# codgodtao/TMDiff

Measured on AMD Instinct MI355X. Metric: UNet denoise-steps/sec (8-ch 64x64, batch 32), higher is better.
Workload: dtype f32; 1 GPU; BASELINE configs[1]: batch-32 8-ch 64x64 tiles, DDPM p_sample steps of the T=1000 cosine schedule, channel_multiplier [32,64,128,256], full UNet forward (both branches) + fused DDPM update per step; batch_per_gpu=32, parallelism=batch-parallel x1, weights=key-hashed random init, text_embedding=fixed synthetic 768-d

## Files before the change

include/tmdiff_hip.h:

```cpp
#ifndef TMDIFF_HIP_H
#define TMDIFF_HIP_H

#include <stddef.h>
#include <stdint.h>

#ifdef __cplusplus
extern "C" {
#endif

#define TMDIFF_ABI_VERSION 6

#define TMDIFF_OK 0
#define TMDIFF_E_INVALID (-1)
#define TMDIFF_E_UNSUPPORTED (-2)
#define TMDIFF_E_LAUNCH (-3)

typedef void* tmdiff_stream_t;

int tmdiff_version(void);
const char* tmdiff_last_error_string(void);

typedef struct tmdiff_conv3d_desc {
  int32_t B, N, H, W;
  int32_t Cin, Cout;
// ... 79 lines not shown
int tmdiff_conv3d_wino_pack_weights_multi(const tmdiff_wino_pack_entry* entries_dev, const int32_t* chunk_tensor_dev,
                                          const int32_t* chunk_index_dev, int32_t n_chunks, tmdiff_stream_t stream);
int tmdiff_conv3d_wino_fwd(const tmdiff_conv3d_desc* d, void* workspace, tmdiff_stream_t stream);
int tmdiff_conv3d_wino_fwd_stage(const tmdiff_conv3d_desc* d, void* workspace, int32_t stage, tmdiff_stream_t stream);
int tmdiff_conv3d_wino_fwd_xp(const tmdiff_conv3d_desc* d, void* workspace, int32_t stage, float* xp_out, tmdiff_stream_t stream);
int tmdiff_conv3d_wino_fwd_planes(const tmdiff_conv3d_desc* d, void* workspace, int32_t stage, float* xp_out, int32_t planes,
                                  tmdiff_stream_t stream);

int tmdiff_conv3d_wf_supported(const tmdiff_conv3d_desc* d);
int64_t tmdiff_conv3d_wf_blocks(const tmdiff_conv3d_desc* d);
size_t tmdiff_conv3d_wf_splitk_workspace_bytes(const tmdiff_conv3d_desc* d);
size_t tmdiff_conv3d_wf_workspace_bytes(const tmdiff_conv3d_desc* d);
int32_t tmdiff_conv3d_wf_plan(int32_t B, int32_t Cin, int32_t Cout, int32_t N, int32_t H, int32_t W, int32_t groups, int32_t llm,
                              int64_t* tiles);
int tmdiff_conv3d_wf_fwd(const tmdiff_conv3d_desc* d, void* workspace, tmdiff_stream_t stream);
int tmdiff_conv3d_wfll_supported(const tmdiff_conv3d_desc* d);
size_t tmdiff_conv3d_wfll_packed_bytes(int32_t Cout, int32_t Cin);
int tmdiff_conv3d_wfll_pack_weights(const float* w, float* packed, int32_t Cout, int32_t Cin, float ll_scale,
                                    tmdiff_stream_t stream);
size_t tmdiff_conv3d_wfll_splitk_workspace_bytes(const tmdiff_conv3d_desc* d);
int tmdiff_conv3d_wfll_fwd(const tmdiff_conv3d_desc* d, float ll_scale, tmdiff_stream_t stream);

size_t tmdiff_conv3d_packed_bf16_bytes(int32_t Cout, int32_t Cin, int32_t ksize, int32_t groups);
int tmdiff_conv3d_pack_weights_bf16(const float* w, void* packed, int32_t Cout, int32_t Cin, int32_t ksize,
                                    int32_t groups, tmdiff_stream_t stream);
int tmdiff_conv3d_pack_weights_bf16_dgrad(const float* w, void* packed, int32_t Cout, int32_t Cin, int32_t ksize,
                                          int32_t groups, tmdiff_stream_t stream);
size_t tmdiff_conv3d_bf16_workspace_bytes(const tmdiff_conv3d_desc* d);
int tmdiff_conv3d_fwd_bf16(const tmdiff_conv3d_desc* d, void* workspace, tmdiff_stream_t stream);

// ... 294 lines not shown
```

tmdiff_amd/Hyper_unet_general.py:

```python
import math

import torch
import torch.nn as nn

from . import ops, routing

PROMPTS = ("QB", "WV3", "GF2", "WV2", "WV4")

def synthetic_text_embeddings(seed=1234):
    out = {}
    for k, name in enumerate(PROMPTS):
        g = torch.Generator(device="cpu").manual_seed(seed + k)
        out[name] = torch.randn(1, 768, generator=g)
    return out


class Swish(nn.Module):

    def forward(self, x):
        raise RuntimeError("Swish is fused into the HIP kernels; it is never called as a module")



_MASK_FN = None
# ... 307 lines not shown
                        prep["w_wino"][name] = {}
        if self.compute_dtype == "fp32" and ops.config.ll_compose:
            for blk in ("down1", "down2", "down3"):
                m = self.get_submodule(blk + ".down.Conv_0")
                if ops.ll_conv_supported(m.out_channels, m.in_channels, m.kernel_size[0], m.groups):
                    prep["w_ll"][blk + ".down.Conv_0"] = ops.pack_conv_weight_ll(m.weight.detach().float().contiguous(), 0.5)
                    if ops.config.winograd and ops.config.wfll and m.out_channels % 32 == 0:
                        prep["w_wfll"][blk + ".down.Conv_0"] = ops.pack_conv_weight_wfll(m.weight.detach().float().contiguous(), 0.5)
        shift, scale = self._projection_layers()
        prep["shift_bank"] = _Bank(shift, dev)
        prep["scale_bank"] = _Bank(scale, dev)
        self._prep = prep
        self._cond = None
        return prep

    def _conv(self, P, name, segs, use_bias=True, bias_scale=1.0, bias=None, emit=False, **kw):
        m = self.get_submodule(name)
        if bias is None:
            bias = m.bias.detach() if (use_bias and m.bias is not None) else None
        if emit:
            kw["emit"] = emit
        math = "bf16" if name in P["bf16"] else "fp32"
        if m.kernel_size[0] != 3:
            out = ops.conv3d(segs, P["w"][name], m.out_channels, m.kernel_size[0], groups=m.groups, math=math, bias=bias,
                             bias_scale=bias_scale, **kw)
            return (out, None) if emit is None else out
        ww = P["w_wino"].get(name)

        def packed(planes):
            if planes not in ww:
                ww[planes] = ops.pack_conv_weight_wino(m.weight.detach().float().contiguous(), groups=m.groups, planes=planes)
            return ww[planes]

        def packed_wf():
            if "wf" not in ww:
                ww["wf"] = ops.pack_conv_weight_wino(m.weight.detach().float().contiguous(), groups=m.groups, mode=2, planes=6)
            return ww["wf"]

        weights = ops.ConvWeights(lambda: P["w"][name], packed_wf if ww is not None else None, packed if ww is not None else None)
        out = ops.conv3d_auto(segs, weights, m.out_channels, groups=m.groups, math=math, bias=bias, bias_scale=bias_scale, **kw)
        return (out, None) if emit is None else out

    def _spec(self, P, S, shift=None, scale=None, act=True):
        d = {"act": act}
        if shift is not None:
            d["shift"], d["shift_stride"] = P["shift_bank"].slot(S["shift"], shift)
        if scale is not None:
            d["scale"], d["scale_stride"] = P["scale_bank"].slot(S["scale"], scale)
        return d

    @staticmethod
    def _own(spec):
        return dict(in_act=spec["act"], in_shift=spec.get("shift"), shift_stride=spec.get("shift_stride", 0),
                    in_scale=spec.get("scale"), scale_stride=spec.get("scale_stride", 0))
# ... 37 lines not shown
        if side is not None:
            t1p = self._conv(P, name + ".conv20", [side], keep_y=False, emit=pro21)
        elif pre is not None:
            t1p = self._conv(P, name + ".conv20", [pre], keep_y=False, emit=pro21, x_bf16_shape=shape if pre.dtype == torch.int16 else None)
        else:
            t1p = self._conv(P, name + ".conv20", segs, keep_y=False, emit=pro21, **self._own(pro20))
        if plan.emit_ll:
            y2, yll = self._conv(P, name + ".conv21", [t1p], use_bias=False, residual=res, keep_y=False, emit=dict(emit, ll=True), **rckw)
            return None, y2, yll, plan.s2d
        y, y2 = self._conv(P, name + ".conv21", [t1p], use_bias=False, residual=res, emit=emit,
                           x_bf16_shape=shape if name + ".conv21" in P["bf16"] else None, **rckw)
        return (y, y2, None, plan.s2d) if want_ll else (y, y2)

    def _conv0(self, P, name, x, pre):
        if pre is None:
            return self._conv(P, name + ".Conv_0", [x], in_act=True)
        return self._conv(P, name + ".Conv_0", [pre], x_bf16_shape=tuple(x.shape[2:]) if pre.dtype == torch.int16 else None)

    def _down(self, P, S, name, x, flag, want_high, pre=None, emit=None, fuse=False, xq=None, s2d=False):
        shape = x.shape if x is not None else (*xq.shape[:3], 2 * xq.shape[3], 2 * xq.shape[4])
        plan = self._down_plan(P, name, shape, not want_high, pre is not None and pre.dtype == torch.float32, s2d, fuse)
        pro = self._spec(P, S, shift=None if flag else name + ".Dense_0", scale=name + ".dense1")
        if plan.conv0 == "dwt":
            hll, *bands = self._conv(P, name + ".Conv_0", [pre], keep_y=False, emit=dict(pro, dwt=True))
        elif plan.conv0 is None:
            hh = self._conv0(P, name, x, pre)
        rc2 = {}
        if not ops.config.conv2_after_ll:
            xll = ops.haar_dwt2d(self._conv(P, name + ".Conv_2", [x]), want_high=False, ll_scale=0.5)[0]
        else:
            if xq is None:
                xq = ops.haar_dwt2d(x, want_high=False, ll_scale=0.5)[0]
# ... 242 lines not shown
```

tmdiff_amd/_lib.py:

```python
import ctypes as C
import os

_HERE = os.path.dirname(os.path.abspath(__file__))
LIB_PATH = os.environ.get("TMDIFF_HIP_LIB") or os.path.join(_HERE, "libtmdiff_hip.so")

c_float_p = C.POINTER(C.c_float)
vp = C.c_void_p


class Conv3dDesc(C.Structure):
    _fields_ = [
        ("B", C.c_int32), ("N", C.c_int32), ("H", C.c_int32), ("W", C.c_int32),
        ("Cin", C.c_int32), ("Cout", C.c_int32),
        ("groups", C.c_int32), ("ksize", C.c_int32), ("nseg", C.c_int32),
        ("seg_c", C.c_int32 * 3),
        ("seg_x", vp * 3),
        ("w_packed", vp), ("bias", vp), ("bias_scale", C.c_float),
        ("in_shift", vp), ("in_scale", vp), ("in_shift_stride", C.c_int32), ("in_scale_stride", C.c_int32),
        ("in_mask", vp), ("in_act", C.c_int32),
        ("residual", vp), ("out_scale", C.c_float),
        ("y", vp),
        ("y2", vp), ("y2_shift", vp), ("y2_scale", vp), ("y2_shift_stride", C.c_int32), ("y2_scale_stride", C.c_int32),
        ("y2_act", C.c_int32), ("y2_bf16", C.c_int32), ("x_bf16", C.c_int32),
        ("splitk_ws", vp), ("splitk_ws_bytes", C.c_int64),
# ... 15 lines not shown
    "tmdiff_conv3d_fwd_staged_workspace_bytes": (C.c_size_t, [C.POINTER(Conv3dDesc)]),
    "tmdiff_conv3d_fwd_staged": (C.c_int, [C.POINTER(Conv3dDesc), vp, vp]),
    "tmdiff_conv3d_wino_supported": (C.c_int, [C.POINTER(Conv3dDesc)]),
    "tmdiff_conv3d_wino_blocks": (C.c_int64, [C.POINTER(Conv3dDesc)]),
    "tmdiff_conv3d_wino_workspace_bytes": (C.c_size_t, [C.POINTER(Conv3dDesc)]),
    "tmdiff_conv3d_wino_planes": (C.c_int32, [C.c_int32]),
    "tmdiff_conv3d_wino_packed_bytes": (C.c_size_t, [C.c_int32, C.c_int32, C.c_int32, C.c_int32]),
    "tmdiff_conv3d_wino_pack_weights": (C.c_int, [vp, vp, C.c_int32, C.c_int32, C.c_int32, C.c_int32, C.c_int32, vp]),
    "tmdiff_conv3d_wino_pack_weights_multi_chunk": (C.c_int32, []),
    "tmdiff_conv3d_wino_pack_weights_multi": (C.c_int, [vp, vp, vp, C.c_int32, vp]),
    "tmdiff_conv3d_wf_supported": (C.c_int, [C.POINTER(Conv3dDesc)]),
    "tmdiff_conv3d_wf_blocks": (C.c_int64, [C.POINTER(Conv3dDesc)]),
    "tmdiff_conv3d_wf_workspace_bytes": (C.c_size_t, [C.POINTER(Conv3dDesc)]),
    "tmdiff_conv3d_wf_splitk_workspace_bytes": (C.c_size_t, [C.POINTER(Conv3dDesc)]),
    "tmdiff_conv3d_wf_fwd": (C.c_int, [C.POINTER(Conv3dDesc), vp, vp]),
    "tmdiff_conv3d_wino_fwd": (C.c_int, [C.POINTER(Conv3dDesc), vp, vp]),
    "tmdiff_conv3d_wino_fwd_planes": (C.c_int, [C.POINTER(Conv3dDesc), vp, C.c_int32, vp, C.c_int32, vp]),
    "tmdiff_conv3d_wino_fwd_xp": (C.c_int, [C.POINTER(Conv3dDesc), vp, C.c_int32, vp, vp]),
    "tmdiff_conv3d_wino_fwd_stage": (C.c_int, [C.POINTER(Conv3dDesc), vp, C.c_int32, vp]),
    "tmdiff_conv3d_prologue_fwd": (C.c_int, [C.POINTER(Conv3dDesc), vp, vp]),
    "tmdiff_conv3d_ll_supported": (C.c_int, [C.POINTER(Conv3dDesc)]),
    "tmdiff_conv3d_ll_splitk_workspace_bytes": (C.c_size_t, [C.POINTER(Conv3dDesc)]),
    "tmdiff_conv3d_ll_packed_bytes": (C.c_size_t, [C.c_int32, C.c_int32]),
    "tmdiff_conv3d_ll_pack_weights": (C.c_int, [vp, vp, C.c_int32, C.c_int32, C.c_float, vp]),
    "tmdiff_conv3d_ll_fwd": (C.c_int, [C.POINTER(Conv3dDesc), C.c_float, vp]),
    "tmdiff_conv3d_packed_bf16_bytes": (C.c_size_t, [C.c_int32, C.c_int32, C.c_int32, C.c_int32]),
    "tmdiff_conv3d_pack_weights_bf16": (C.c_int, [vp, vp, C.c_int32, C.c_int32, C.c_int32, C.c_int32, vp]),
    "tmdiff_conv3d_bf16_workspace_bytes": (C.c_size_t, [C.POINTER(Conv3dDesc)]),
    "tmdiff_conv3d_fwd_bf16": (C.c_int, [C.POINTER(Conv3dDesc), vp, vp]),
    "tmdiff_conv3d_wgrad_workspace_bytes": (C.c_size_t, [C.POINTER(Conv3dDesc)]),
# ... 185 lines not shown
```

tmdiff_amd/csrc/bufaddr.h:

```cpp
#pragma once
#include <hip/hip_runtime.h>

namespace tmdiff {
namespace buf {

constexpr unsigned kOutside = 0xFFFFFFF0u;

#if defined(__HIP_DEVICE_COMPILE__)
using rsrc = __amdgpu_buffer_rsrc_t;
__device__ __forceinline__ rsrc make(const void* base, unsigned bytes) {
  return __builtin_amdgcn_make_buffer_rsrc(const_cast<void*>(base), 0, bytes, 0x00020000);
}
using u32x4 = __attribute__((ext_vector_type(4))) unsigned;
using u32x2 = __attribute__((ext_vector_type(2))) unsigned;
__device__ __forceinline__ float load(rsrc r, unsigned voff, unsigned soff) {
  return __uint_as_float(__builtin_amdgcn_raw_buffer_load_b32(r, voff, soff, 0));
}
__device__ __forceinline__ float4 load4(rsrc r, unsigned voff) {
  const u32x4 v = __builtin_amdgcn_raw_buffer_load_b128(r, voff, 0, 0);
  return make_float4(__uint_as_float(v.x), __uint_as_float(v.y), __uint_as_float(v.z), __uint_as_float(v.w));
}
__device__ __forceinline__ void store4(rsrc r, unsigned voff, float4 t) {
  const u32x4 v = {__float_as_uint(t.x), __float_as_uint(t.y), __float_as_uint(t.z), __float_as_uint(t.w)};
  __builtin_amdgcn_raw_buffer_store_b128(v, r, voff, 0, 0);
}
__device__ __forceinline__ void store4(rsrc r, unsigned voff, uint4 t) {
  const u32x4 v = {t.x, t.y, t.z, t.w};
  __builtin_amdgcn_raw_buffer_store_b128(v, r, voff, 0, 0);
}
__device__ __forceinline__ void store2(rsrc r, unsigned voff, float2 t) {
  const u32x2 v = {__float_as_uint(t.x), __float_as_uint(t.y)};
  __builtin_amdgcn_raw_buffer_store_b64(v, r, voff, 0, 0);
}
__device__ __forceinline__ void dma_b128(rsrc r, unsigned voff, unsigned soff, float* dst) {
  __builtin_amdgcn_raw_ptr_buffer_load_lds(r, dst, 16, voff, soff, 0, 0);
}
#else
struct rsrc {};
__device__ __forceinline__ rsrc make(const void*, unsigned) { return {}; }
__device__ __forceinline__ float load(rsrc, unsigned, unsigned) { return 0.f; }
__device__ __forceinline__ float4 load4(rsrc, unsigned) { return make_float4(0.f, 0.f, 0.f, 0.f); }
__device__ __forceinline__ void store4(rsrc, unsigned, float4) {}
__device__ __forceinline__ void store4(rsrc, unsigned, uint4) {}
__device__ __forceinline__ void store2(rsrc, unsigned, float2) {}
__device__ __forceinline__ void dma_b128(rsrc, unsigned, unsigned, float*) {}
#endif
__device__ __forceinline__ unsigned at(unsigned base, unsigned add) { return base >= kOutside ? kOutside : base + add; }

__device__ __forceinline__ void dma_b32(const float* src, float* dst) {
#if defined(__HIP_DEVICE_COMPILE__)
  __builtin_amdgcn_global_load_lds(src, dst, 4, 0, 0);
#endif
}
__device__ __forceinline__ void dma_b128(const float* src, float* dst) {
#if defined(__HIP_DEVICE_COMPILE__)
  __builtin_amdgcn_global_load_lds(src, dst, 16, 0, 0);
// ... 6 lines not shown
```

tmdiff_amd/ops.py:

```python
import collections
import ctypes as C
import math
import os

import numpy as np
import torch

from . import _lib, routing
from ._lib import Conv3dDesc, check, lib



class KernelConfig:

    _FLAG = lambda default: (lambda v: (v != "0") if default else (v == "1"))
    _FIELDS = {
        "winograd": ("TMDIFF_WINOGRAD", _FLAG(True), True), "wf": ("TMDIFF_WF", _FLAG(True), True),
        "wf_pair": ("TMDIFF_WF_PAIR", _FLAG(True), True), "wf_splitk": ("TMDIFF_WF_SPLITK", _FLAG(True), True),
        "wf_min_fill": ("TMDIFF_WF_MIN_FILL", float, 0.7), "wino_min_blocks": ("TMDIFF_WINO_MIN_BLOCKS", int, 256),
        "ll_compose": ("TMDIFF_LL_COMPOSE", _FLAG(True), True), "wfll": ("TMDIFF_WFLL", _FLAG(True), True),
        "train_ll_wino": ("TMDIFF_TRAIN_LL_WINO", _FLAG(True), True),
        "conv2_after_ll": ("TMDIFF_CONV2_AFTER_LL", _FLAG(True), True),
        "epilogue_fuse": ("TMDIFF_EPILOGUE_FUSE", _FLAG(True), True), "producer_fuse": ("TMDIFF_PRODUCER_FUSE", _FLAG(True), True),
        "fp32_staged": ("TMDIFF_FP32_STAGED", str, "auto"), "bf16_pack": ("TMDIFF_BF16_PACK", str, "auto"),
        "wgrad_wino": ("TMDIFF_WGRAD_WINO", _FLAG(True), True), "wgrad_wino_bias": ("TMDIFF_WGRAD_WINO_BIAS", _FLAG(True), True),
        "wgrad_bias": ("TMDIFF_WGRAD_BIAS", _FLAG(False), False), "wino_multipack": ("TMDIFF_WINO_MULTIPACK", _FLAG(True), True),
        "fuse_res_conv": ("TMDIFF_FUSE_RES_CONV", _FLAG(True), True), "emit_ll": ("TMDIFF_EMIT_LL", _FLAG(True), True),
        "emit_dwt": ("TMDIFF_EMIT_DWT", _FLAG(True), True), "side_xp": ("TMDIFF_SIDE_XP", _FLAG(True), True),
        "train_fused_resblock": ("TMDIFF_TRAIN_FUSED_RESBLOCK", _FLAG(True), True),
        "train_graph": ("TMDIFF_TRAIN_GRAPH", _FLAG(False), False),
        "train_two_streams": ("TMDIFF_TRAIN_STREAMS", _FLAG(True), True),
        "sample_graph": ("TMDIFF_SAMPLE_GRAPH", _FLAG(False), False),
        "grad_bf16": ("TMDIFF_GRAD_BF16", _FLAG(False), False),
    }

    def __init__(self, env=None):
        env = os.environ if env is None else env
        for name, (var, parse, default) in self._FIELDS.items():
            object.__setattr__(self, name, parse(env[var]) if var in env else default)

    def __setattr__(self, name, value):
        if name not in self._FIELDS:
            raise AttributeError(f"ops.config has no switch {name!r}")
        object.__setattr__(self, name, value)

    def key(self):
        return tuple(getattr(self, n) for n in self._FIELDS)

# ... 519 lines not shown
        raise ValueError(f"pack_conv_weight_wino: weight shape {tuple(w.shape)} (groups {groups}, mode {mode}, planes {planes}) not supported")
    out = torch.empty(nb // 4, device=w.device, dtype=torch.float32)
    check(lib.tmdiff_conv3d_wino_pack_weights(_chk(w.detach(), "w"), out.data_ptr(), cout, cin, groups, mode, planes, stream_ptr()),
          "conv3d_wino_pack_weights")
    return out


wino_conv_supported = routing.wino_weight_ok
ll_conv_supported = routing.ll_weight_ok
wf_route = routing.wf_route
wfll_route = routing.wfll_route


class ConvWeights:

    def __init__(self, direct, wf=None, wino=None):
        self.direct, self.wf, self.wino = direct, wf, wino


def conv3d_auto(segs, weights, cout, groups=1, math="fp32", emit=None, keep_y=True, xp_out=None, x_bf16_shape=None, family=None,
                **kw):
    if math == "bf16" or x_bf16_shape is not None:
        return conv3d(segs, weights.direct(), cout, 3, groups=groups, math=math, emit=emit, keep_y=keep_y,
                      x_bf16_shape=x_bf16_shape, **kw)
    b, _, n, h, w = segs[0].shape
    cin = sum(s_.shape[1] for s_ in segs)
    masked, dropout, plain = kw.get("in_mask") is not None, kw.get("drop") is not None, _plain(segs, kw)
    fam = family or routing.conv3_family(b, cin, cout, n, h, w, groups, plain=plain, masked=masked, dropout=dropout,
                                         keep_xp=xp_out is not None)
    if fam in ("wf", "wf_pair") and weights.wf is not None:
        return conv3d_wf(segs, weights.wf(), cout, emit=emit, keep_y=keep_y, groups=groups, xp_out=xp_out, **kw)
    if fam in ("wino4", "wino2") and weights.wino is not None:
        from . import fallback
        planes = 6 if fam == "wino4" else 4
        return fallback.conv3d_wino(segs, weights.wino(planes), cout, planes, emit=emit, keep_y=keep_y, groups=groups,
                                    xp_out=xp_out, **kw)
    if (emit is not None and (emit.get("s2d") or emit.get("ll") or emit.get("dwt"))) or kw.get("res_conv") is not None:
        raise ValueError("conv3d_auto: only conv3d_wf writes a space-to-depth second output / folds a residual convolution "
                         "(ask routing.wf_route first)")
    if fam not in ("staged", "fused"):
        fam = routing.direct_family(cin, cout, groups, plain, masked, dropout, xp_out is not None, extents=(b, n, h, w))
    return conv3d(segs, weights.direct(), cout, 3, groups=groups, staged=fam == "staged", emit=emit, keep_y=keep_y,
                  xp_out=xp_out, **kw)

# ... 18 lines not shown
    y_hi = [torch.empty(*q, device=dev, dtype=torch.float32) for _ in range(3)] if want_dwt else None
    y, y2 = _outputs("conv3d_wf", dev, (b, cout, n, h, w), keep_y, emit,
                     None if want_dwt else ((b, 4 * cout, n, h // 2, w // 2) if s2d else (b, cout, n, h, w)))
    d = make_conv_desc(segs, w_packed, cout, 3, y, y2=y2, groups=groups, y2_s2d=s2d, y_ll=y_ll, y_hi=y_hi, **kw,
                       **_emit_kw(emit))
    if not lib.tmdiff_conv3d_wf_supported(C.byref(d)):
        raise ValueError("conv3d_wf: shape not supported")
    _lend_splitk(d, dev, lib.tmdiff_conv3d_wf_splitk_workspace_bytes(C.byref(d)) if (config.wf_splitk and not want_ll) else 0)
    nws = lib.tmdiff_conv3d_wf_workspace_bytes(C.byref(d))
    ws = _xp_target("conv3d_wf", xp_out, nws, dev)
    if xp_out is not None and not nws:
        xp_out.copy_(segs[0] if len(segs) == 1 else torch.cat(segs, 1))
    flops = 2.0 * b * cout * ((d.Cin // groups) * 13.5 + d.rc_cin) * n * h * w
    _launch(lib.tmdiff_conv3d_wf_fwd, d, (ws,), "conv3d_wf_fwd", "conv3d_wf_fwd", flops, 3, f" +rc{d.rc_cin}" if d.rc_cin else "")
    return (y_ll, *y_hi) if want_dwt else (y2, y_ll) if want_ll else _result(y, y2)


def pack_conv_weight_ll(w, ll_scale=0.5):
    cout, cin = w.shape[0], w.shape[1]
    nb = lib.tmdiff_conv3d_ll_packed_bytes(cout, cin)
    if tuple(w.shape[2:]) != (3, 3, 3) or nb == 0:
        raise ValueError(f"pack_conv_weight_ll: weight shape {tuple(w.shape)} not supported")
    out = torch.empty(nb // 4, device=w.device, dtype=torch.float32)
    check(lib.tmdiff_conv3d_ll_pack_weights(_chk(w.detach(), "w"), out.data_ptr(), cout, cin, float(ll_scale), stream_ptr()),
          "conv3d_ll_pack_weights")
    return out


def conv3d_ll(x, w_packed, cout, ll_scale=0.5, emit=None, keep_y=True, **kw):
    b, _, n, h, w = x.shape
# ... 1454 lines not shown
```

tmdiff_amd/routing.py:

```python
import collections
import ctypes as C

from . import _lib
from ._lib import lib

PRODUCT_FAMILIES = ("wf", "wf_pair", "wfll", "ll", "staged", "fused", "bf16")
FALLBACK_FAMILIES = ("wino4", "wino2")


def _config():
    from . import ops
    return ops.config


def _grad_bf16():
    return bool(getattr(_config(), "grad_bf16", False))


def wino_weight_ok(cout, cin, ksize=3, groups=1):
    return (ksize == 3 and groups in (1, 3) and cin % groups == 0 and cout % groups == 0 and (cin // groups) % 2 == 0 and
            (cout // groups) % 32 == 0)


def staged_weight_ok(cout, cin, groups=1):
# ... 44 lines not shown
def supported(query, b, cin, cout, n, h, w, groups=1, **fields):
    key = (query, b, cin, cout, n, h, w, groups, tuple(sorted(fields.items())))
    r = _QUERIES.get(key)
    if r is None:
        if len(_QUERIES) > 4096:
            _QUERIES.clear()
        seg_c = cin if isinstance(cin, tuple) else (cin,)
        d = _lib.Conv3dDesc()
        d.B, d.N, d.H, d.W, d.Cin, d.Cout, d.groups, d.ksize, d.nseg = b, n, h, w, sum(seg_c), cout, groups, 3, len(seg_c)
        for i, c in enumerate(seg_c):
            d.seg_c[i] = c
        for k, v in fields.items():
            setattr(d, k, v)
        r = _QUERIES[key] = bool(getattr(lib, query)(C.byref(d)))
    return r


def wfll_route(b, cin, cout, n, h, w):
    if not (_config().wfll and n in (4, 8) and h % 2 == 0 and w % 8 == 0 and cout % 32 == 0):
        return False
    return wf_route(b, 4 * cin, cout, n, h // 2, w // 2, llm=True)[0]


def wino_plan(b, cout, n, h, w, groups=1, cin=None):
    planes = lib.tmdiff_conv3d_wino_planes(int(n))
    if not planes or w % 4:
        return 0, 0
    if cin is not None and not supported("tmdiff_conv3d_wino_supported", b, cin, cout, n, h, w, groups):
        return 0, 0
    cg = cout // groups
# ... 411 lines not shown
```

Baseline: 45.33 batch32-steps/s.

## Add 2D Winograd F(4,3)xF(2,3) conv path for deep low-resolution layers

Adds a new three-pass convolution for fp32 3x3x3 layers with Cin>=128 and Cout>=256 at small spatial sizes (W<=16, H<=32). It applies Winograd transforms along depth (F(4,3)) and width (F(2,3)), runs 24 batched MFMA GEMMs over channels with double-buffered LDS staging, and does the inverse transform plus bias, residual and activation in an output pass. Routing sends eligible 'wf' family convs there by default. The aim is to cut multiply work on the deep UNet layers, at the cost of extra workspace round-trips through global memory, two more kernel launches per conv, and a one-time weight pack.

New measurement: 46.02 batch32-steps/s (median of 6 runs). +1.5%, better.

```diff
diff --git a/include/tmdiff_hip.h b/include/tmdiff_hip.h
--- a/include/tmdiff_hip.h
+++ b/include/tmdiff_hip.h
@@ -117,6 +117,12 @@
 int32_t tmdiff_conv3d_wf_plan(int32_t B, int32_t Cin, int32_t Cout, int32_t N, int32_t H, int32_t W, int32_t groups, int32_t llm,
                               int64_t* tiles);
 int tmdiff_conv3d_wf_fwd(const tmdiff_conv3d_desc* d, void* workspace, tmdiff_stream_t stream);
+
+int tmdiff_conv3d_w2_supported(const tmdiff_conv3d_desc* d);
+size_t tmdiff_conv3d_w2_workspace_bytes(const tmdiff_conv3d_desc* d);
+size_t tmdiff_conv3d_w2_packed_bytes(int32_t Cout, int32_t Cin);
+int tmdiff_conv3d_w2_pack_weights(const float* w, float* packed, int32_t Cout, int32_t Cin, tmdiff_stream_t stream);
+int tmdiff_conv3d_w2_fwd(const tmdiff_conv3d_desc* d, void* workspace, int32_t stages, tmdiff_stream_t stream);
 int tmdiff_conv3d_wfll_supported(const tmdiff_conv3d_desc* d);
 size_t tmdiff_conv3d_wfll_packed_bytes(int32_t Cout, int32_t Cin);
 int tmdiff_conv3d_wfll_pack_weights(const float* w, float* packed, int32_t Cout, int32_t Cin, float ll_scale,
diff --git a/tmdiff_amd/Hyper_unet_general.py b/tmdiff_amd/Hyper_unet_general.py
--- a/tmdiff_amd/Hyper_unet_general.py
+++ b/tmdiff_amd/Hyper_unet_general.py
@@ -345,7 +345,7 @@
         self._cond = None
         return prep
 
-    def _conv(self, P, name, segs, use_bias=True, bias_scale=1.0, bias=None, emit=False, **kw):
+    def _conv(self, P, name, segs, use_bias=True, bias_scale=1.0, bias=None, emit=False, w2=True, **kw):
         m = self.get_submodule(name)
         if bias is None:
             bias = m.bias.detach() if (use_bias and m.bias is not None) else None
@@ -368,7 +368,13 @@
                 ww["wf"] = ops.pack_conv_weight_wino(m.weight.detach().float().contiguous(), groups=m.groups, mode=2, planes=6)
             return ww["wf"]
 
-        weights = ops.ConvWeights(lambda: P["w"][name], packed_wf if ww is not None else None, packed if ww is not None else None)
+        def packed_w2():
+            if "w2" not in ww:
+                ww["w2"] = ops.pack_conv_weight_w2(m.weight.detach().float().contiguous())
+            return ww["w2"]
+
+        weights = ops.ConvWeights(lambda: P["w"][name], packed_wf if ww is not None else None, packed if ww is not None else None,
+                                  packed_w2 if (w2 and ww is not None and m.groups == 1) else None)
         out = ops.conv3d_auto(segs, weights, m.out_channels, groups=m.groups, math=math, bias=bias, bias_scale=bias_scale, **kw)
         return (out, None) if emit is None else out
 
@@ -436,8 +442,8 @@
 
     def _conv0(self, P, name, x, pre):
         if pre is None:
-            return self._conv(P, name + ".Conv_0", [x], in_act=True)
-        return self._conv(P, name + ".Conv_0", [pre], x_bf16_shape=tuple(x.shape[2:]) if pre.dtype == torch.int16 else None)
+            return self._conv(P, name + ".Conv_0", [x], in_act=True, w2=False)
+        return self._conv(P, name + ".Conv_0", [pre], x_bf16_shape=tuple(x.shape[2:]) if pre.dtype == torch.int16 else None, w2=False)
 
     def _down(self, P, S, name, x, flag, want_high, pre=None, emit=None, fuse=False, xq=None, s2d=False):
         shape = x.shape if x is not None else (*xq.shape[:3], 2 * xq.shape[3], 2 * xq.shape[4])
diff --git a/tmdiff_amd/_lib.py b/tmdiff_amd/_lib.py
--- a/tmdiff_amd/_lib.py
+++ b/tmdiff_amd/_lib.py
@@ -53,6 +53,11 @@
     "tmdiff_conv3d_wf_workspace_bytes": (C.c_size_t, [C.POINTER(Conv3dDesc)]),
     "tmdiff_conv3d_wf_splitk_workspace_bytes": (C.c_size_t, [C.POINTER(Conv3dDesc)]),
     "tmdiff_conv3d_wf_fwd": (C.c_int, [C.POINTER(Conv3dDesc), vp, vp]),
+    "tmdiff_conv3d_w2_supported": (C.c_int, [C.POINTER(Conv3dDesc)]),
+    "tmdiff_conv3d_w2_workspace_bytes": (C.c_size_t, [C.POINTER(Conv3dDesc)]),
+    "tmdiff_conv3d_w2_packed_bytes": (C.c_size_t, [C.c_int32, C.c_int32]),
+    "tmdiff_conv3d_w2_pack_weights": (C.c_int, [vp, vp, C.c_int32, C.c_int32, vp]),
+    "tmdiff_conv3d_w2_fwd": (C.c_int, [C.POINTER(Conv3dDesc), vp, C.c_int32, vp]),
     "tmdiff_conv3d_wino_fwd": (C.c_int, [C.POINTER(Conv3dDesc), vp, vp]),
     "tmdiff_conv3d_wino_fwd_planes": (C.c_int, [C.POINTER(Conv3dDesc), vp, C.c_int32, vp, C.c_int32, vp]),
     "tmdiff_conv3d_wino_fwd_xp": (C.c_int, [C.POINTER(Conv3dDesc), vp, C.c_int32, vp, vp]),
diff --git a/tmdiff_amd/csrc/bufaddr.h b/tmdiff_amd/csrc/bufaddr.h
--- a/tmdiff_amd/csrc/bufaddr.h
+++ b/tmdiff_amd/csrc/bufaddr.h
@@ -20,6 +20,13 @@
   const u32x4 v = __builtin_amdgcn_raw_buffer_load_b128(r, voff, 0, 0);
   return make_float4(__uint_as_float(v.x), __uint_as_float(v.y), __uint_as_float(v.z), __uint_as_float(v.w));
 }
+__device__ __forceinline__ float2 load2(rsrc r, unsigned voff) {
+  const u32x2 v = __builtin_amdgcn_raw_buffer_load_b64(r, voff, 0, 0);
+  return make_float2(__uint_as_float(v.x), __uint_as_float(v.y));
+}
+__device__ __forceinline__ void store(rsrc r, unsigned voff, float t) {
+  __builtin_amdgcn_raw_buffer_store_b32(__float_as_uint(t), r, voff, 0, 0);
+}
 __device__ __forceinline__ void store4(rsrc r, unsigned voff, float4 t) {
   const u32x4 v = {__float_as_uint(t.x), __float_as_uint(t.y), __float_as_uint(t.z), __float_as_uint(t.w)};
   __builtin_amdgcn_raw_buffer_store_b128(v, r, voff, 0, 0);
@@ -40,6 +47,8 @@
 __device__ __forceinline__ rsrc make(const void*, unsigned) { return {}; }
 __device__ __forceinline__ float load(rsrc, unsigned, unsigned) { return 0.f; }
 __device__ __forceinline__ float4 load4(rsrc, unsigned) { return make_float4(0.f, 0.f, 0.f, 0.f); }
+__device__ __forceinline__ float2 load2(rsrc, unsigned) { return make_float2(0.f, 0.f); }
+__device__ __forceinline__ void store(rsrc, unsigned, float) {}
 __device__ __forceinline__ void store4(rsrc, unsigned, float4) {}
 __device__ __forceinline__ void store4(rsrc, unsigned, uint4) {}
 __device__ __forceinline__ void store2(rsrc, unsigned, float2) {}
diff --git a/tmdiff_amd/csrc/conv3d_w2.hip b/tmdiff_amd/csrc/conv3d_w2.hip
--- /dev/null
+++ b/tmdiff_amd/csrc/conv3d_w2.hip
@@ -0,0 +1,438 @@
+#include "bufaddr.h"
+#include "common.h"
+
+namespace {
+
+using namespace tmdiff;
+
+constexpr int W2_XP = 384;
+constexpr int W2_NP = 256;
+constexpr int W2_KC = 16;
+constexpr int W2_CO = 64;
+
+struct W2Plan {
+  int T, Q, TW, Hp, IP, OP;
+  int G, ptiles;
+  size_t xh_floats, mh_floats;
+};
+
+bool w2_shape_ok(const tmdiff_conv3d_desc* d) {
+  if (!d || d->ksize != 3 || d->groups != 1 || d->x_bf16 || d->y2_bf16 || d->nseg != 1) return false;
+  if (d->B <= 0 || (d->N != 4 && d->N != 8) || d->W < 2 || d->W > 16 || d->W % 2 || d->H < 4 || d->H > 32) return false;
+  if (d->Cin < 128 || d->Cin % 32 || d->Cout < 256 || d->Cout % W2_CO || d->seg_c[0] != d->Cin) return false;
+  if (d->in_mask || d->drop_p > 0.f || d->rc_x || d->rc_cin || d->y_ll || d->y_hi[0] || d->y2_s2d || d->xp_out) return false;
+  return true;
+}
+
+W2Plan w2_plan(const tmdiff_conv3d_desc* d) {
+  W2Plan p;
+  p.T = d->N / 4; p.Q = d->B * p.T; p.TW = d->W / 2; p.Hp = d->H + 2;
+  p.IP = p.Hp * p.TW; p.OP = d->H * p.TW;
+  p.G = W2_NP / p.OP < W2_XP / p.IP ? W2_NP / p.OP : W2_XP / p.IP;
+  if (p.G > p.Q) p.G = p.Q;
+  p.ptiles = (p.Q + p.G - 1) / p.G;
+  p.xh_floats = (size_t)24 * d->Cin * p.Q * p.IP;
+  p.mh_floats = (size_t)24 * d->Cout * p.Q * p.OP;
+  return p;
+}
+
+bool w2_fits(const tmdiff_conv3d_desc* d, const W2Plan& p) {
+  const size_t xk = p.xh_floats / 24 * 4, mk = p.mh_floats / 24 * 4, uk = (size_t)3 * d->Cin * d->Cout * 4;
+  return xk < (1ull << 31) && mk < (1ull << 31) && uk < (1ull << 31) && p.Q <= 65535 &&
+         (long)p.ptiles * (d->Cout / W2_CO) * 24 < 0x7fffffffL;
+}
+
+__global__ void __launch_bounds__(256) w2_pack_kernel(const float* __restrict__ w, float* __restrict__ u, int Cout, int Cin) {
+#pragma clang fp contract(off)
+  const long idx = (long)blockIdx.x * 256 + threadIdx.x;
+  if (idx >= (long)3 * Cin * Cout) return;
+  const int e = idx & 3;
+  long r = idx >> 2;
+  const int co = r % Cout; r /= Cout;
+  const int cq = r % (Cin / 4);
+  const int dh = r / (Cin / 4);
+  const int ci = cq * 4 + e;
+  const float* src = w + ((long)co * Cin + ci) * 27 + dh * 3;
+  float t[6][3];
+#pragma unroll
+  for (int dw = 0; dw < 3; ++dw) {
+    const float g0 = src[dw], g1 = src[9 + dw], g2 = src[18 + dw];
+    const float s02 = g0 + g2;
+    const float ev = g0 + 4.f * g2, od = 2.f * g1;
+    t[0][dw] = 0.25f * g0;
+    t[1][dw] = (s02 + g1) * (-1.f / 6.f);
+    t[2][dw] = (g1 - s02) * (1.f / 6.f);
+    t[3][dw] = (ev + od) * (1.f / 24.f);
+    t[4][dw] = (ev - od) * (1.f / 24.f);
+    t[5][dw] = g2;
+  }
+  const long plane = (long)3 * Cin * Cout;
+  float* dst = u + (((long)dh * (Cin / 4) + cq) * Cout + co) * 4 + e;
+#pragma unroll
+  for (int kb = 0; kb < 6; ++kb) {
+    const float s02 = t[kb][0] + t[kb][2];
+    dst[(kb * 4 + 0) * plane] = t[kb][0];
+    dst[(kb * 4 + 1) * plane] = 0.5f * (s02 + t[kb][1]);
+    dst[(kb * 4 + 2) * plane] = 0.5f * (s02 - t[kb][1]);
+    dst[(kb * 4 + 3) * plane] = t[kb][2];
+  }
+}
+
+struct W2InArgs {
+  const float* x;
+  float* xh;
+  const float* in_shift;
+  const float* in_scale;
+  int shift_stride, scale_stride, in_act;
+  int Cin, N, H, W, T, TW, IP;
+  long QIP;
+};
+
+__global__ void __launch_bounds__(256) w2_input_kernel(const W2InArgs a) {
+  __shared__ float tile[24 * 8 * 33];
+  const int tid = threadIdx.x;
+  const int cc = blockIdx.x, hp = blockIdx.y, q = blockIdx.z;
+  const int b = q / a.T, t = q % a.T;
+  const int h = hp - 1;
+  {
+    const int c = tid >> 3, tw = tid & 7;
+    const int ch = cc * 32 + c;
+    const long hw = (long)a.H * a.W;
+    const bool ok = h >= 0 && h < a.H && tw < a.TW;
+    const float sh = a.in_shift ? a.in_shift[(long)b * a.shift_stride + ch] : 0.f;
+    const float sc = a.in_scale ? a.in_scale[(long)b * a.scale_stride + ch] : 1.f;
+    const float* src = a.x + ((long)b * a.Cin + ch) * a.N * hw + (long)h * a.W + 2 * tw;
+    float d[6][4];
+#pragma unroll
+    for (int j = 0; j < 6; ++j) {
+      const int n = 4 * t - 1 + j;
+      float2 v = make_float2(0.f, 0.f);
+      if (ok && n >= 0 && n < a.N) {
+        v = *reinterpret_cast<const float2*>(src + (long)n * hw);
+        v.x += sh, v.y += sh;
+        if (a.in_act) v.x = silu_f(v.x), v.y = silu_f(v.y);
+        v.x *= sc, v.y *= sc;
+      }
+      const float left = __shfl_up(v.y, 1, 8), right = __shfl_down(v.x, 1, 8);
+      d[j][0] = tw == 0 ? 0.f : left;
+      d[j][1] = v.x, d[j][2] = v.y;
+      d[j][3] = tw == 7 ? 0.f : right;
+    }
+    float o[6][4];
+#pragma unroll
+    for (int e = 0; e < 4; ++e) {
+      const float d0 = d[0][e], d1 = d[1][e], d2 = d[2][e], d3 = d[3][e], d4 = d[4][e], d5 = d[5][e];
+      const float a42 = d4 - 4.f * d2, b31 = d3 - 4.f * d1, c42 = d4 - d2, e31 = d3 - d1;
+      o[0][e] = (4.f * d0 + d4) - 5.f * d2;
+      o[1][e] = a42 + b31;
+      o[2][e] = a42 - b31;
+      o[3][e] = c42 + 2.f * e31;
+      o[4][e] = c42 - 2.f * e31;
+      o[5][e] = (4.f * d1 + d5) - 5.f * d3;
+    }
+#pragma unroll
+    for (int kb = 0; kb < 6; ++kb) {
+      float* dst = tile + (kb * 4 * 8 + tw) * 33 + c;
+      dst[0 * 8 * 33] = o[kb][0] - o[kb][2];
+      dst[1 * 8 * 33] = o[kb][1] + o[kb][2];
+      dst[2 * 8 * 33] = o[kb][2] - o[kb][1];
+      dst[3 * 8 * 33] = o[kb][1] - o[kb][3];
+    }
+  }
+  __syncthreads();
+  const int n_out = 24 * 8 * a.TW;
+  const long pos = (long)q * a.IP + (long)hp * a.TW;
+  for (int i = tid; i < n_out; i += 256) {
+    const int tw = i % a.TW, r = i / a.TW;
+    const int cq = r & 7, k = r >> 3;
+    const float* s = tile + (k * 8 + tw) * 33 + cq * 4;
+    float* dst = a.xh + (((long)k * (a.Cin / 4) + cc * 8 + cq) * a.QIP + pos + tw) * 4;
+    *reinterpret_cast<float4*>(dst) = make_float4(s[0], s[1], s[2], s[3]);
+  }
+}
+
+struct W2GemmArgs {
+  const float* xh;
+  const float* u;
+  float* mh;
+  int Cin, Cout, Q, TW, IP, OP, G, ptiles, cotiles;
+  unsigned total_blocks;
+};
+
+__global__ void __launch_bounds__(256, 2) w2_gemm_kernel(const W2GemmArgs a) {
+  constexpr int XS = W2_XP * W2_KC;
+  constexpr int US = 3 * W2_KC * W2_CO;
+  constexpr int STAGE = XS + US;
+  __shared__ __attribute__((aligned(16))) float lds[2 * STAGE];
+  float* const st0 = lds;
+  float* const st1 = lds + STAGE;
+
+  const int tid = threadIdx.x;
+  const int lane = tid & 63, wv = __builtin_amdgcn_readfirstlane(tid >> 6);
+  const int l31 = lane & 31, khalf = lane >> 5;
+
+  unsigned id = xcd_remap(blockIdx.x, a.total_blocks);
+  const int co_t = take(id, a.cotiles);
+  const int p_t = take(id, a.ptiles);
+  const int k = __builtin_amdgcn_readfirstlane(id);
+  const int q0 = p_t * a.G;
+  const int nvalid = min(a.G, a.Q - q0) * a.OP;
+  const long QIP = (long)a.Q * a.IP, QOP = (long)a.Q * a.OP;
+  const long xplane = (long)a.Cin * QIP, uplane = (long)3 * a.Cin * a.Cout, mplane = QOP * a.Cout;
+  const buf::rsrc rx = buf::make(a.xh + (long)k * xplane, (unsigned)(xplane * 4));
+  const buf::rsrc ru = buf::make(a.u + (long)k * uplane, (unsigned)(uplane * 4));
+  const buf::rsrc rm = buf::make(a.mh + (long)k * mplane, (unsigned)(mplane * 4));
+
+  unsigned xv[6], uv[3];
+#pragma unroll
+  for (int c = 0; c < 6; ++c) xv[c] = (unsigned)((q0 * a.IP + c * 64 + lane) * 16);
+  const unsigned quad_bytes = (unsigned)(QIP * 16);
+#pragma unroll
+  for (int i = 0; i < 3; ++i) {
+    const int ui = wv * 3 + i, dh = ui >> 2, qd = ui & 3;
+    uv[i] = (unsigned)((((long)dh * (a.Cin / 4) + qd) * a.Cout + co_t * W2_CO + lane) * 16);
+  }
+  const unsigned ustage_bytes = (unsigned)(4 * a.Cout * 16);
+  auto issue = [&](int s, float* st) __attribute__((always_inline)) {
+    const unsigned xso = (unsigned)(4 * s + wv) * quad_bytes, uso = (unsigned)s * ustage_bytes;
+#pragma unroll
+    for (int c = 0; c < 6; ++c) buf::dma_b128(rx, xv[c], xso, st + (wv * W2_XP + c * 64) * 4);
+#pragma unroll
+    for (int i = 0; i < 3; ++i) buf::dma_b128(ru, uv[i], uso, st + XS + (wv * 3 + i) * 256);
+  };
+
+  int aoff[2][3];
+#pragma unroll
+  for (int pb = 0; pb < 2; ++pb) {
+    int c = (2 * wv + pb) * 32 + l31;
+    if (c >= nvalid) c = 0;
+    const int padded = (c / a.OP) * a.IP + c % a.OP;
+#pragma unroll
+    for (int dh = 0; dh < 3; ++dh) aoff[pb][dh] = (khalf * W2_XP + padded + dh * a.TW) * 4;
+  }
+  const int boff = XS + (khalf * W2_CO + l31) * 4;
+
+  f32x16 acc[2][2];
+#pragma unroll
+  for (int pb = 0; pb < 2; ++pb)
+#pragma unroll
+    for (int cb = 0; cb < 2; ++cb)
+#pragma unroll
+      for (int r = 0; r < 16; ++r) acc[pb][cb][r] = 0.f;
+
+  auto compute = [&](const float* st) __attribute__((always_inline)) {
+    static_for<0, 6>([&](auto ic) __attribute__((always_inline)) {
+      constexpr int dh = decltype(ic)::value / 2, m = decltype(ic)::value % 2;
+      float4 av[2], bv[2];
+#pragma unroll
+      for (int pb = 0; pb < 2; ++pb) av[pb] = *reinterpret_cast<const float4*>(st + aoff[pb][dh] + m * 2 * W2_XP * 4);
+#pragma unroll
+      for (int cb = 0; cb < 2; ++cb)
+        bv[cb] = *reinterpret_cast<const float4*>(st + boff + ((dh * 4 + 2 * m) * W2_CO + cb * 32) * 4);
+#pragma unroll
+      for (int e = 0; e < 4; ++e) {
+        const float a0 = e == 0 ? av[0].x : e == 1 ? av[0].y : e == 2 ? av[0].z : av[0].w;
+        const float a1 = e == 0 ? av[1].x : e == 1 ? av[1].y : e == 2 ? av[1].z : av[1].w;
+        const float b0 = e == 0 ? bv[0].x : e == 1 ? bv[0].y : e == 2 ? bv[0].z : bv[0].w;
+        const float b1 = e == 0 ? bv[1].x : e == 1 ? bv[1].y : e == 2 ? bv[1].z : bv[1].w;
+        acc[0][0] = __builtin_amdgcn_mfma_f32_32x32x2f32(a0, b0, acc[0][0], 0, 0, 0);
+        acc[0][1] = __builtin_amdgcn_mfma_f32_32x32x2f32(a0, b1, acc[0][1], 0, 0, 0);
+        acc[1][0] = __builtin_amdgcn_mfma_f32_32x32x2f32(a1, b0, acc[1][0], 0, 0, 0);
+        acc[1][1] = __builtin_amdgcn_mfma_f32_32x32x2f32(a1, b1, acc[1][1], 0, 0, 0);
+      }
+    });
+  };
+
+  const int ns = a.Cin / W2_KC;
+  issue(0, st0);
+  for (int s = 0; s < ns; s += 2) {
+    __builtin_amdgcn_s_waitcnt(0x0F70);
+    __syncthreads();
+    issue(s + 1, st1);
+    compute(st0);
+    __builtin_amdgcn_s_waitcnt(0x0F70);
+    __syncthreads();
+    if (s + 2 < ns) issue(s + 2, st0);
+    compute(st1);
+  }
+
+#pragma unroll
+  for (int pb = 0; pb < 2; ++pb)
+#pragma unroll
+    for (int r = 0; r < 16; ++r) {
+      const int c = (2 * wv + pb) * 32 + (r & 3) + 8 * (r >> 2) + 4 * khalf;
+      const unsigned o = c < nvalid ? (unsigned)((((long)q0 * a.OP + c) * a.Cout + co_t * W2_CO + l31) * 4) : buf::kOutside;
+      buf::store(rm, o, acc[pb][0][r]);
+      buf::store(rm, buf::at(o, 128u), acc[pb][1][r]);
+    }
+}
+
+struct W2OutArgs {
+  const float* mh;
+  const float* bias;
+  float bias_scale;
+  const float* residual;
+  float out_scale;
+  float* y;
+  float* y2;
+  const float* y2_shift;
+  const float* y2_scale;
+  int y2_shift_stride, y2_scale_stride, y2_act;
+  int Cout, N, H, W, T, TW, OP;
+  long QOP;
+};
+
+template <bool Y, bool RES, bool Y2>
+__global__ void __launch_bounds__(256) w2_output_kernel(const W2OutArgs a) {
+#pragma clang fp contract(off)
+  __shared__ float tile[4 * 32 * 17];
+  const int tid = threadIdx.x;
+  const int cc = blockIdx.x, h = blockIdx.y, q = blockIdx.z;
+  const int b = q / a.T, t = q % a.T;
+  {
+    const int co_l = tid & 31, tw = tid >> 5;
+    if (tw < a.TW) {
+      const float* src = a.mh + ((long)q * a.OP + h * a.TW + tw) * a.Cout + cc * 32 + co_l;
+      const long kstride = a.QOP * a.Cout;
+      float r[6][2];
+#pragma unroll
+      for (int kb = 0; kb < 6; ++kb) {
+        const float m0 = src[(kb * 4 + 0) * kstride], m1 = src[(kb * 4 + 1) * kstride], m2 = src[(kb * 4 + 2) * kstride],
+                    m3 = src[(kb * 4 + 3) * kstride];
+        r[kb][0] = (m0 + m1) + m2;
+        r[kb][1] = (m1 - m2) - m3;
+      }
+#pragma unroll
+      for (int j = 0; j < 2; ++j) {
+        const float p12 = r[1][j] + r[2][j], d12 = r[1][j] - r[2][j], p34 = r[3][j] + r[4][j], d34 = r[3][j] - r[4][j];
+        float* dst = tile + co_l * 17 + 2 * tw + j;
+        dst[0 * 32 * 17] = (r[0][j] + p12) + p34;
+        dst[1 * 32 * 17] = d12 + 2.f * d34;
+        dst[2 * 32 * 17] = p12 + 4.f * p34;
+        dst[3 * 32 * 17] = (d12 + 8.f * d34) + r[5][j];
+      }
+    }
+  }
+  __syncthreads();
+  const long plane = (long)a.N * a.H * a.W;
+  const long cb = ((long)b * a.Cout + cc * 32) * plane;
+  const unsigned span = (unsigned)(32 * plane * 4);
+  const buf::rsrc ry = buf::make(Y ? a.y + cb : nullptr, Y ? span : 0u);
+  const buf::rsrc rr = buf::make(RES ? a.residual + cb : nullptr, RES ? span : 0u);
+  const buf::rsrc r2 = buf::make(Y2 ? a.y2 + cb : nullptr, Y2 ? span : 0u);
+#pragma unroll
+  for (int it = 0; it < 4; ++it) {
+    const int i = tid + 256 * it;
+    const int wp = i & 7, band = (i >> 3) & 3, co_l = i >> 5;
+    const int co = cc * 32 + co_l;
+    const unsigned o = wp < a.TW ? (unsigned)(((co_l * (long)a.N + 4 * t + band) * a.H + h) * a.W + 2 * wp) * 4u : buf::kOutside;
+    const float* s = tile + (band * 32 + co_l) * 17 + 2 * wp;
+    float v[2] = {s[0], s[1]};
+    const float bias_t = a.bias ? a.bias[co] * a.bias_scale : 0.f;
+    float2 res = make_float2(0.f, 0.f);
+    if constexpr (RES) res = buf::load2(rr, o);
+    v[0] = (v[0] + bias_t + res.x) * a.out_scale;
+    v[1] = (v[1] + bias_t + res.y) * a.out_scale;
+    if constexpr (Y) buf::store2(ry, o, make_float2(v[0], v[1]));
+    if constexpr (Y2) {
+      const float sh2 = a.y2_shift ? a.y2_shift[(long)b * a.y2_shift_stride + co] : 0.f;
+      const float sc2 = a.y2_scale ? a.y2_scale[(long)b * a.y2_scale_stride + co] : 1.f;
+      float u[2];
+#pragma unroll
+      for (int e = 0; e < 2; ++e) {
+        const float x = v[e] + sh2;
+        const float xa = silu_f(x);
+        u[e] = (a.y2_act ? xa : x) * sc2;
+      }
+      buf::store2(r2, o, make_float2(u[0], u[1]));
+    }
+  }
+}
+
+}
+
+extern "C" int tmdiff_conv3d_w2_supported(const tmdiff_conv3d_desc* d) {
+  return w2_shape_ok(d) && w2_fits(d, w2_plan(d)) ? 1 : 0;
+}
+
+extern "C" size_t tmdiff_conv3d_w2_workspace_bytes(const tmdiff_conv3d_desc* d) {
+  if (!w2_shape_ok(d)) return 0;
+  const W2Plan p = w2_plan(d);
+  return (p.xh_floats + p.mh_floats) * sizeof(float);
+}
+
+extern "C" size_t tmdiff_conv3d_w2_packed_bytes(int32_t Cout, int32_t Cin) {
+  if (Cout <= 0 || Cin <= 0 || Cin % 4) return 0;
+  return (size_t)72 * Cout * Cin * sizeof(float);
+}
+
+extern "C" int tmdiff_conv3d_w2_pack_weights(const float* w, float* packed, int32_t Cout, int32_t Cin, tmdiff_stream_t stream) {
+  using namespace tmdiff;
+  TMDIFF_REQUIRE(w && packed, "conv3d_w2_pack_weights: NULL pointer");
+  TMDIFF_REQUIRE(Cout > 0 && Cin > 0 && Cin % 4 == 0 && (size_t)72 * Cout * Cin < (1ull << 31),
+                 "conv3d_w2_pack_weights: Cout=%d Cin=%d (Cin %% 4 == 0)", Cout, Cin);
+  const long n = (long)3 * Cin * Cout;
+  w2_pack_kernel<<<(unsigned)((n + 255) / 256), 256, 0, as_stream(stream)>>>(w, packed, Cout, Cin);
+  return check_launch("conv3d_w2_pack_weights");
+}
+
+extern "C" int tmdiff_conv3d_w2_fwd(const tmdiff_conv3d_desc* d, void* workspace, int32_t stages, tmdiff_stream_t stream) {
+  using namespace tmdiff;
+  TMDIFF_REQUIRE(d && workspace, "conv3d_w2_fwd: NULL pointer");
+  if (!w2_shape_ok(d))
+    return fail(TMDIFF_E_UNSUPPORTED, "conv3d_w2_fwd: fp32 3x3x3, groups 1, one input tensor, 4 or 8 bands, even W <= 16, 4 <= H <= 32, "
+                                      "Cin >= 128 (%% 32), Cout >= 256 (%% 64), plain y / y2 / residual epilogue");
+  const W2Plan p = w2_plan(d);
+  if (!w2_fits(d, p)) return fail(TMDIFF_E_UNSUPPORTED, "conv3d_w2_fwd: tensor too large for 32-bit offsets");
+  TMDIFF_REQUIRE(d->seg_x[0] && d->w_packed && (d->y || d->y2), "conv3d_w2_fwd: input, weights and an output");
+  TMDIFF_REQUIRE(aligned16(d->seg_x[0]) && aligned16(workspace) && aligned16(d->w_packed) && aligned16(d->y) && aligned16(d->y2) &&
+                     aligned16(d->residual),
+                 "conv3d_w2_fwd: 16-byte aligned tensors / workspace");
+  hipStream_t st = as_stream(stream);
+  float* xh = static_cast<float*>(workspace);
+  float* mh = xh + p.xh_floats;
+  if (stages == 0) stages = 7;
+
+  if (stages & 1) {
+    W2InArgs a;
+    a.x = d->seg_x[0]; a.xh = xh;
+    a.in_shift = d->in_shift; a.in_scale = d->in_scale;
+    a.shift_stride = bank_stride(d->in_shift_stride, d->Cin);
+    a.scale_stride = bank_stride(d->in_scale_stride, d->Cin);
+    a.in_act = d->in_act;
+    a.Cin = d->Cin; a.N = d->N; a.H = d->H; a.W = d->W; a.T = p.T; a.TW = p.TW; a.IP = p.IP;
+    a.QIP = (long)p.Q * p.IP;
+    w2_input_kernel<<<dim3((unsigned)(d->Cin / 32), (unsigned)p.Hp, (unsigned)p.Q), 256, 0, st>>>(a);
+    if (const int rc = check_launch("conv3d_w2_fwd(input pass)")) return rc;
+  }
+  if (stages & 2) {
+    W2GemmArgs a;
+    a.xh = xh; a.u = d->w_packed; a.mh = mh;
+    a.Cin = d->Cin; a.Cout = d->Cout; a.Q = p.Q; a.TW = p.TW; a.IP = p.IP; a.OP = p.OP; a.G = p.G; a.ptiles = p.ptiles;
+    a.cotiles = d->Cout / W2_CO;
+    if (const int rc = set_grid(a, (long)p.ptiles * a.cotiles * 24, "conv3d_w2_fwd")) return rc;
+    w2_gemm_kernel<<<a.total_blocks, 256, 0, st>>>(a);
+    if (const int rc = check_launch("conv3d_w2_fwd")) return rc;
+  }
+  if (stages & 4) {
+    W2OutArgs a;
+    a.mh = mh;
+    a.bias = d->bias; a.bias_scale = d->bias_scale; a.residual = d->residual; a.out_scale = d->out_scale;
+    a.y = d->y; a.y2 = d->y2; a.y2_shift = d->y2_shift; a.y2_scale = d->y2_scale; a.y2_act = d->y2_act;
+    a.y2_shift_stride = bank_stride(d->y2_shift_stride, d->Cout);
+    a.y2_scale_stride = bank_stride(d->y2_scale_stride, d->Cout);
+    a.Cout = d->Cout; a.N = d->N; a.H = d->H; a.W = d->W; a.T = p.T; a.TW = p.TW; a.OP = p.OP;
+    a.QOP = (long)p.Q * p.OP;
+    const dim3 grid((unsigned)(d->Cout / 32), (unsigned)d->H, (unsigned)p.Q);
+#define TMDIFF_W2_OUT(Y, R, Y2) w2_output_kernel<Y, R, Y2><<<grid, 256, 0, st>>>(a)
+    if (d->y) {
+      if (d->residual) { if (d->y2) TMDIFF_W2_OUT(true, true, true); else TMDIFF_W2_OUT(true, true, false); }
+      else             { if (d->y2) TMDIFF_W2_OUT(true, false, true); else TMDIFF_W2_OUT(true, false, false); }
+    } else {
+      if (d->residual) TMDIFF_W2_OUT(false, true, true); else TMDIFF_W2_OUT(false, false, true);
+    }
+#undef TMDIFF_W2_OUT
+    if (const int rc = check_launch("conv3d_w2_fwd(output pass)")) return rc;
+  }
+  return TMDIFF_OK;
+}
diff --git a/tmdiff_amd/ops.py b/tmdiff_amd/ops.py
--- a/tmdiff_amd/ops.py
+++ b/tmdiff_amd/ops.py
@@ -32,6 +32,7 @@
         "train_two_streams": ("TMDIFF_TRAIN_STREAMS", _FLAG(True), True),
         "sample_graph": ("TMDIFF_SAMPLE_GRAPH", _FLAG(False), False),
         "grad_bf16": ("TMDIFF_GRAD_BF16", _FLAG(False), False),
+        "wino2d": ("TMDIFF_WINO2D", _FLAG(True), True),
     }
 
     def __init__(self, env=None):
@@ -581,8 +582,8 @@
 
 class ConvWeights:
 
-    def __init__(self, direct, wf=None, wino=None):
-        self.direct, self.wf, self.wino = direct, wf, wino
+    def __init__(self, direct, wf=None, wino=None, w2=None):
+        self.direct, self.wf, self.wino, self.w2 = direct, wf, wino, w2
 
 
 def conv3d_auto(segs, weights, cout, groups=1, math="fp32", emit=None, keep_y=True, xp_out=None, x_bf16_shape=None, family=None,
@@ -595,6 +596,11 @@
     masked, dropout, plain = kw.get("in_mask") is not None, kw.get("drop") is not None, _plain(segs, kw)
     fam = family or routing.conv3_family(b, cin, cout, n, h, w, groups, plain=plain, masked=masked, dropout=dropout,
                                          keep_xp=xp_out is not None)
+    if (fam in ("wf", "wf_pair") and weights.w2 is not None and family is None and xp_out is None and len(segs) == 1 and
+            not masked and not dropout and kw.get("res_conv") is None and
+            not (emit is not None and (emit.get("s2d") or emit.get("ll") or emit.get("dwt"))) and
+            routing.wino2d_route(b, cin, cout, n, h, w, groups)):
+        return conv3d_w2(segs[0], weights.w2(), cout, emit=emit, keep_y=keep_y, **kw)
     if fam in ("wf", "wf_pair") and weights.wf is not None:
         return conv3d_wf(segs, weights.wf(), cout, emit=emit, keep_y=keep_y, groups=groups, xp_out=xp_out, **kw)
     if fam in ("wino4", "wino2") and weights.wino is not None:
@@ -643,6 +649,31 @@
     flops = 2.0 * b * cout * ((d.Cin // groups) * 13.5 + d.rc_cin) * n * h * w
     _launch(lib.tmdiff_conv3d_wf_fwd, d, (ws,), "conv3d_wf_fwd", "conv3d_wf_fwd", flops, 3, f" +rc{d.rc_cin}" if d.rc_cin else "")
     return (y_ll, *y_hi) if want_dwt else (y2, y_ll) if want_ll else _result(y, y2)
+
+
+def pack_conv_weight_w2(w):
+    cout, cin = w.shape[0], w.shape[1]
+    nb = lib.tmdiff_conv3d_w2_packed_bytes(cout, cin)
+    if tuple(w.shape[2:]) != (3, 3, 3) or nb == 0:
+        raise ValueError(f"pack_conv_weight_w2: weight shape {tuple(w.shape)} not supported")
+    out = torch.empty(nb // 4, device=w.device, dtype=torch.float32)
+    check(lib.tmdiff_conv3d_w2_pack_weights(_chk(w.detach(), "w"), out.data_ptr(), cout, cin, stream_ptr()), "conv3d_w2_pack_weights")
+    return out
+
+
+def conv3d_w2(x, w_packed, cout, emit=None, keep_y=True, stages=0, **kw):
+    b, _, n, h, w = x.shape
+    dev = x.device
+    if emit is not None and (emit.get("s2d") or emit.get("ll") or emit.get("dwt")):
+        raise ValueError("conv3d_w2: no space-to-depth / LL / Haar outputs (conv3d_wf writes those)")
+    y, y2 = _outputs("conv3d_w2", dev, (b, cout, n, h, w), keep_y, emit, (b, cout, n, h, w))
+    d = make_conv_desc([x], w_packed, cout, 3, y, y2=y2, **kw, **_emit_kw(emit))
+    if not lib.tmdiff_conv3d_w2_supported(C.byref(d)):
+        raise ValueError("conv3d_w2: shape not supported (routing.wino2d_ok)")
+    nws = lib.tmdiff_conv3d_w2_workspace_bytes(C.byref(d))
+    ws = _workspace(dev, nws, "w2").data_ptr()
+    _launch(lib.tmdiff_conv3d_w2_fwd, d, (ws, int(stages)), "conv3d_w2_fwd", "conv3d_w2_fwd", 2.0 * b * cout * d.Cin * 9.0 * n * h * w)
+    return _result(y, y2)
 
 
 def pack_conv_weight_ll(w, ll_scale=0.5):
diff --git a/tmdiff_amd/routing.py b/tmdiff_amd/routing.py
--- a/tmdiff_amd/routing.py
+++ b/tmdiff_amd/routing.py
@@ -82,6 +82,22 @@
             setattr(d, k, v)
         r = _QUERIES[key] = bool(getattr(lib, query)(C.byref(d)))
     return r
+
+
+def wino2d_ok(b, cin, cout, n, h, w, groups=1):
+    if groups != 1 or b <= 0 or n not in (4, 8) or w < 2 or w > 16 or w % 2 or h < 4 or h > 32:
+        return False
+    if cin < 128 or cin % 32 or cout < 256 or cout % 64:
+        return False
+    q, tw = b * (n // 4), w // 2
+    ip, op = (h + 2) * tw, h * tw
+    g = max(1, min(q, 256 // op, 384 // ip))
+    return (4 * cin * q * ip < (1 << 31) and 4 * cout * q * op < (1 << 31) and 12 * cin * cout < (1 << 31) and q <= 65535 and
+            ((q + g - 1) // g) * (cout // 64) * 24 < 0x7fffffff)
+
+
+def wino2d_route(b, cin, cout, n, h, w, groups=1):
+    return bool(_config().wino2d and wino2d_ok(b, cin, cout, n, h, w, groups))
 
 
 def wfll_route(b, cin, cout, n, h, w):
```
